# ChenWu98/cycle-diffusion

Measured on AMD Instinct MI355X. Metric: images/sec, SD-v1.4 512px CycleDiffusion 100+100 steps, 1/2/4/8 MI355X, higher is better.
Workload: dtype fp16; 1 GPU; C2: Stable-Diffusion-v1.4-shaped U-Net + KL-f8 VAE, 512x512, custom_steps=99 white_box_steps=100 eta=0.1 skip 0, 1 trial, encoder scale 1, decoder CFG 3; batch_per_gpu=4, global_batch=4, parallelism=dp1, steps_per_launch_set=5, launch_set_cap=16, launch_sets_in_flight_per_gpu=1, images_in_flight_per_gpu=20, distributed=single process, weights=synthetic(seed=0)

## Files before the change

### cycle-diffusion_amd/_ffi.py

```python
import ctypes as C
import os

import numpy as np

_HERE = os.path.dirname(os.path.abspath(__file__))
LIB_PATH = os.path.join(_HERE, "lib", "libcyclediff.so")

CD_NET_UNET_OPENAI, CD_NET_UNET_HO, CD_NET_VAE_KL, CD_NET_CLIP_TEXT, CD_NET_BERT_XTR = 1, 2, 3, 4, 5
CD_NET_OCLIP_TEXT, CD_NET_OCLIP_VISION, CD_NET_INCEPTION_FID, CD_NET_LPIPS = 6, 7, 8, 9
CD_SCHED_DDIM, CD_SCHED_DDPM = 0, 1
CD_PREC_16, CD_PREC_F32, CD_PREC_F32X3 = 0, 1, 2
CD_MASK_QSAMPLE, CD_MASK_ENCODER = 0, 1
MASK_SOURCES = {"q_sample": CD_MASK_QSAMPLE, "encoder": CD_MASK_ENCODER}
ACT_NONE, ACT_SILU, ACT_GELU, ACT_GEGLU, ACT_QGELU, ACT_RELU = 0, 1, 2, 3, 4, 5


class NetDesc(C.Structure):
    _fields_ = [
        ("kind", C.c_int), ("image_size", C.c_int), ("in_channels", C.c_int), ("out_channels", C.c_int),
        ("model_channels", C.c_int), ("num_res_blocks", C.c_int),
        ("n_mult", C.c_int), ("channel_mult", C.c_int * 8),
        ("n_attn", C.c_int), ("attn", C.c_int * 8),
        ("num_heads", C.c_int), ("num_head_channels", C.c_int),
        ("use_spatial_transformer", C.c_int), ("context_dim", C.c_int), ("transformer_depth", C.c_int),
# ... 78 lines not shown
    "cd_vae_encode": [_VP, _I, _VP, _VP, _U64, _I, _I, _I, _F, _VP],
    "cd_vae_decode": [_VP, _I, _VP, _I, _I, _F, _F, _F, _VP],
    "cd_vae_encode_hw": [_VP, _I, _VP, _VP, _U64, _I, _I, _I, _I, _F, _VP],
    "cd_vae_decode_hw": [_VP, _I, _VP, _I, _I, _I, _F, _F, _F, _VP],
    "cd_dpm_encode": [_VP, _I, _I, _VP, _VP, _VP, _I, _F, _I, _I, _VP, _VP, _U64, _I, _VP],
    "cd_ddim_decode": [_VP, _I, _I, _VP, _I, _I, _VP, _VP, _I, _F, _I, _I, _VP, _VP, _U64, _VP],
    "cd_ddim_decode_v": [_VP, _I, _I, _VP, _I, _I, _VP, _VP, _I, _VP, _I, _I, _VP, _VP, _U64, _VP],
    "cd_ddim_invert": [_VP, _I, _I, _VP, _VP, _VP, _I, _F, _I, _I, _VP, _VP, _VP],
    "cd_cycle_translate": [_VP, C.POINTER(TranslateArgs)],
    "cd_ddim_decode_masked": [_VP, _I, _I, _VP, _I, _I, _VP, _VP, _I, _F, _VP, _I, _I, _VP, _VP, _U64, _VP, _VP, _I, _I, _VP, _VP,
                              _U64, _VP],
    "cd_ilvr_decode": [_VP, _I, _I, _VP, _I, _I, _I, _I, _VP, _VP, _U64, _VP, _I, _I, _I, _VP, _VP, _U64, _VP],
    "cd_automask": [_VP, _I, _VP, _VP, _VP, _I, _I, _I, _I, _F, _F, _VP, _U64, _I, _F, _F, _I, _VP, _VP],
    "cd_word_maps": [_VP, _I, _VP, _VP, _I, _I, _VP, _I, _I, _I, _I, _F, _F, _VP, _U64, _I, _I, _I, _VP, C.POINTER(_I)],
    "cd_pix_refine": [_VP, _I, _I, _VP, _I, _I, _VP, _VP, _U64],
    "cd_op_pack_conv_weight": [_VP, _VP, _I, _I, _I, _I, _I, C.POINTER(_VP), C.POINTER(_I), C.POINTER(_I)],
    "cd_op_free": [_VP, _VP],
    "cd_op_conv2d": [_VP, _VP, _I, _VP, _I, _I, _I, _I, _VP, _I, _I, _I, _I, _I, _I, _I, _VP, _VP, _VP, _I, _I, _VP],
    "cd_op_conv2d_16": [_VP, _VP, _I, _VP, _I, _I, _I, _I, _VP, _I, _I, _I, _I, _I, _I, _I, _VP, _VP, _VP, _I, _I, _VP,
                        _VP],
    "cd_op_last_gemm_config": [_VP] + [C.POINTER(_I)] * 5,
    "cd_op_up_phase_reorder": [_VP, _VP, _I, _I, _I, _I, _VP],
    "cd_op_groupnorm": [_VP, _VP, _I, _I, _I, _I, _I, _F, _VP, _VP, _VP, _I, _VP],
    "cd_op_groupnorm_ex": [_VP, _VP, _I, _I, _VP, _I, _I, _I, _I, _I, _F, _VP, _VP, _VP, _I, _I, _VP, _VP, _I, _VP],
    "cd_op_pack_conv_weight_prec": [_VP, _VP, _I, _I, _I, _I, _I, C.POINTER(_VP)],
    "cd_op_conv2d_prec": [_VP, _VP, _I, _I, _VP, _I, _I, _I, _I, _I, _VP, _I, _I, _I, _I, _I, _I, _I, _VP, _VP, _I, _VP, _I, _I,
                          _I, _I, _I, _I, _F, _VP, _VP],
    "cd_op_attention_prec": [_VP, _VP, _VP, _VP, _I, _I, _I, _I, _I, _I, _I, _I, _F, _I, _VP, _I, _I, _VP],
    "cd_op_rows_prec": [_VP, _I, _VP, _I64, _I, _I, _VP, _I, _I, _VP, _VP, _I, _VP],
    "cd_op_resample_prec": [_VP, _I, _VP, _I, _I, _I, _I, _I, _VP],
    "cd_op_layernorm": [_VP, _VP, _I, _I, _VP, _VP, _F, _VP],
    "cd_op_st_entry": [_VP, _VP, _I, _I, _I, _VP, _VP, _F, _VP, _VP, _VP, _VP, _VP, _VP, _VP, _I, _VP, _VP, _VP,
                       C.POINTER(_I)],
    "cd_op_attention": [_VP, _VP, _VP, _VP, _I, _I, _I, _I, _I, _F, _I, _VP],
    "cd_op_cross_attention_ctrl": [_VP, _VP, _VP, _VP, _VP, _VP, _VP, _VP, _VP, _I, _I, _I, _I, _I, _I, _I, _I, _F, _VP],
    "cd_op_cross_attention_ctrl_ex": [_VP, _VP, _VP, _VP, _VP, _VP, _VP, _VP, _VP, _I, _I, _I, _I, _I, _I, _I, _I, _F, _I, _I,
                                      _VP],
    "cd_op_cross_attention_maps": [_VP, _VP, _VP, _VP, _I, _I, _I, _I, _I, _I, _I, _I, _F, _I, _VP],
    "cd_op_attention_ex": [_VP, _VP, _VP, _VP, _I, _I, _I, _I, _I, _I, _I, _I, _I, _I, _F, _I, _VP, _I, _I, _VP],
    "cd_op_lowpass": [_VP, _VP, _I, _I, _I, _I, _VP],
    "cd_op_softmax_rows": [_VP, _VP, _I64, _I, _VP],
    "cd_op_timestep_embedding": [_VP, _VP, _I, _I, _I, _VP],
    "cd_op_sched_step": [_VP, _I, _I, _VP, _VP, _VP, _VP, _I, _F, _VP, _VP, _I, _I, _I, _I, _VP],
    "cd_op_gauss": [_VP, _U64, C.c_uint32, _I64, _I64, _VP],
    "cd_op_automask_reduce": [_VP, _VP, _VP, _I, _I, _I, _I, _I, _F, _F, _I, _VP, _VP, _VP],
    "cd_op_local_blend_mask": [_VP, _VP, _VP, _I, _I, _I, _I, _I, _F, _VP],
    "cd_op_sched_step_masked": [_VP, _I, _VP, _VP, _VP, _I, _F, _VP, _VP, _VP, _I, _I, _F, _F, _VP, _I, _I, _I, _I, _VP, _I],
    "cd_op_sega_guidance": [_VP, _VP, _I, _I, _I, _I, _I, _F, _VP, _VP, _I, _F, _F, _VP, _VP, _VP, _VP, _VP],
    "cd_op_window_gather": [_VP, _VP, _VP, _I, _I, _I, _I, _I, _I, _I, _I, _VP],
    "cd_op_window_fuse": [_VP, _VP, _VP, _I, _I, _I, _I, _I, _I, _I, _I, _VP],
    "cd_op_layout": [_VP, _I, _VP, _VP, _I, _I, _I, _I, _I, _F, _F, _I],
    "cd_op_resample16": [_VP, _I, _VP, _VP, _I, _I, _I, _I],
    "cd_op_copy_rows16": [_VP, _VP, _I, _VP, _I, _I64, _I],
    "cd_op_vec_linear": [_VP, _VP, _I, _VP, _VP, _VP, _I, _I, _I, _I, _I, _I],
    "cd_op_tokens": [_VP, _I, _VP, _VP, _VP, _VP, _VP, _I, _I, _I, _I],
    "cd_op_posterior_sample": [_VP, _VP, _I, _VP, _U64, _VP, _I, _I, _I, _F, _I],
    "cd_op_vq_quantize": [_VP, _VP, _F, _VP, _I, _I, _I, _I, _VP, _I],
    "cd_op_gemm_batched": [_VP, _VP, _I, _I64, _VP, _I, _I64, _I, _I, _I, _I, _F, _VP, _VP, _I, _VP, _I, _I, _VP, _I, _I64, _I],
    "cd_op_attn_block_core": [_VP, _VP, _I, _VP, _I, _VP, _VP, _I, _I, _I, _VP, _I, _VP, C.POINTER(_I)],
    "cd_op_pool3x3": [_VP, _VP, _I, _I, _I, _I, _I, _I, _I, _I, _I, _I, _VP],
    "cd_op_global_avg": [_VP, _VP, _I, _I, _I, _I, _VP],
    "cd_op_basic_conv": [_VP, _VP, _I, _I, _I, _I, _I, _VP, _VP, _VP, _VP, _VP, _I, _I, _I, _I, _I, _I, _I, _I, _I, _VP, _VP,
                         _VP],
    "cd_op_lpips_layer": [_VP, _VP, _VP, _VP, _I, _I, _I, _I, _VP],
    "cd_op_pool2x2": [_VP, _VP, _I, _I, _I, _I, _I, _I, _I, _VP],
    "cd_op_bench_conv": [_VP, _I, _I, _I, _I, _I, _I, _I, _I, _I, _I, _I, _I, C.POINTER(C.c_float)],
# ... 53 lines not shown
```

### cycle-diffusion_amd/csrc/capi_internal.h

```cpp
#pragma once
#include <stdlib.h>
#include <string.h>
#include <unistd.h>

#include <map>
#include <utility>

#include "engine.h"

using namespace cd;

struct StepPacer {
  static constexpr int kAhead = 2, kRing = kAhead + 1;
  hipEvent_t ev[kRing] = {nullptr, nullptr, nullptr};
  long n = 0;
  bool enabled = true;
  void init() {
    const char* e = getenv("CYCLEDIFF_HOST_PACING");
    enabled = !(e && e[0] == '0');
    for (auto& x : ev) HIP_CHECK(hipEventCreateWithFlags(&x, hipEventBlockingSync | hipEventDisableTiming));
  }
  static void sleep_until_done(hipEvent_t e) {
    for (;;) {
      const hipError_t q = hipEventQuery(e);
// ... 15 lines not shown
    ++n;
  }
  void destroy() { for (auto& x : ev) if (x) { (void)hipEventDestroy(x); x = nullptr; } }
};

struct CoefStaging {
  static constexpr int kSlots = 4;
  static constexpr size_t kSlotBytes = 64 << 10;
  char* host = nullptr;
  hipEvent_t done[kSlots] = {nullptr, nullptr, nullptr, nullptr};
  int next = 0;
  void init() {
    HIP_CHECK(hipHostMalloc((void**)&host, kSlots * kSlotBytes, hipHostMallocDefault));
    for (auto& x : done) HIP_CHECK(hipEventCreateWithFlags(&x, hipEventBlockingSync | hipEventDisableTiming));
  }
  void destroy() {
    for (auto& x : done) if (x) { (void)hipEventDestroy(x); x = nullptr; }
    if (host) { (void)hipHostFree(host); host = nullptr; }
  }
};

struct cd_engine {
  hipStream_t st = nullptr;
  StepPacer pacer;
  CoefStaging coef_staging;
  Arena arena;
  bf16_t* zeros = nullptr;
  float* gn_partial = nullptr;
  size_t gn_partial_floats = 0;
  std::vector<std::unique_ptr<Net>> nets;
  std::vector<ParamStore*> op_stores;
  ParamStore op_params;
  std::map<std::pair<const void*, const void*>, std::pair<ConvW*, ConvW*>> op_st_entry;
  ParamStore op_params_f32;
  std::unique_ptr<KernelProfiler> prof;
  SplitKWorkspace splitk;
  int* overflow_host = nullptr;
  int* overflow_dev = nullptr;
  void check_overflow() {
    if (overflow_host && *(volatile int*)overflow_host) {
      *(volatile int*)overflow_host = 0;
      CD_CHECK(false, "CD_PREC_F32X3: a GroupNorm output or weight left the fp16 range of the split representation "
                      "(|x| >= 4094 or |w| >= 255); results since the last synchronisation are invalid - run this "
                      "network with CD_PREC_F32");
    }
  }
  Ctx ctx() {
    Ctx c; c.st = st; c.arena = &arena; c.zeros = zeros; c.gn_partial = gn_partial;
    c.gn_partial_floats = gn_partial_floats; c.overflow = overflow_dev;
    return c;
  }
};

struct ArenaScope {
  Arena& a;
  size_t m;
  explicit ArenaScope(Arena& arena) : a(arena), m(arena.mark()) {}
  ~ArenaScope() { a.release(m); }
  ArenaScope(const ArenaScope&) = delete;
  ArenaScope& operator=(const ArenaScope&) = delete;
};

void set_last_error(const char* what);

inline void enter_engine(cd_engine* h) {
  if (!h) return;
// ... 45 lines not shown
```

### cycle-diffusion_amd/csrc/capi_ops.hip

```cpp
#include "capi_internal.h"

namespace {

bf16_t* op_rows16(cd_engine* h, const float* src, int64_t rows, int C) {
  bf16_t* d = (bf16_t*)h->arena.alloc((size_t)rows * C * 2);
  launch_nchw_to_nhwc(h->st, src, d, (int)rows, C, 1, C, 1.f, 0.f, 0);
  return d;
}
Act op_image16(Ctx& c, const float* x, int B, int C, int H, int W, int Cpad) {
  Act a = alloc_act(c, B, H, W, Cpad);
  launch_nchw_to_nhwc(c.st, x, a.p, B, C, H * W, Cpad, 1.f, 0.f, 0);
  return a;
}

bf16_t* op_nan_rows16(cd_engine* h, int64_t rows, int ld) {
  const size_t bytes = (size_t)(rows + 64) * ld * 2;
  bf16_t* t = (bf16_t*)h->arena.alloc(bytes);
  HIP_CHECK(hipMemsetAsync(t, 0xFF, bytes, h->st));
  return t;
}
float* op_nan_buffer(cd_engine* h, size_t n) {
  float* t = (float*)h->arena.alloc(n * sizeof(float));
  launch_fill_f32(h->st, t, __builtin_nanf(""), (int64_t)n);
  return t;
// ... 279 lines not shown
               B > 0 && H > 0 && W > 0, "bad argument");
  ArenaScope arena_scope(h->arena);
  Ctx c = h->ctx();
  const int C = 320, T = H * W;
  ConvW win = *(const ConvW*)w_in;
  win.b = const_cast<float*>(b_in);
  StEntryW w;
  w.norm.g = const_cast<float*>(gn_gamma); w.norm.b = const_cast<float*>(gn_beta); w.norm.C = C; w.norm.eps = gn_eps;
  w.ln1.g = const_cast<float*>(ln_gamma); w.ln1.b = const_cast<float*>(ln_beta); w.ln1.C = C;
  w.proj_in = &win; w.qk1 = (const ConvW*)w_qk; w.v1 = (const ConvW*)w_v;
  CD_CHECK(win.N == C && win.Cpad == C && w.qk1->N == 2 * C && w.qk1->Cpad == C && w.v1->N == C && w.v1->Cpad == C,
           "transformer entry: 320-channel weights expected");
  w.vbias = v_bias;
  {
    const auto key = std::make_pair(w_qk, w_v);
    auto it = h->op_st_entry.find(key);
    if (it == h->op_st_entry.end()) {
      st_entry_alloc(h->op_params, w);
      it = h->op_st_entry.emplace(key, std::make_pair(w.qkv, w.qkv_ln)).first;
    }
    w.qkv = it->second.first; w.qkv_ln = it->second.second;
  }
  st_entry_refresh(h->st, w);
  Act a = op_image16(c, x, B, C, H, W, C);
  if (stages < 0) stages = st_entry_stages();
  const StEntryOut r = st_entry_fwd(c, w, a, stages);
  if (stages_run) *stages_run = r.stages;
  op_download_nchw(h, r.h.p, false, r.h.ld, h_out, B, C, T);
  op_download_nchw(h, r.qk.p, false, r.qk.ld, qk_out, B, 2 * C, T);
  op_download_nchw(h, r.vt, false, r.Tpad, vt_out, B * C, r.Tpad, 1);
  CD_API_END
}

int cd_op_attention(cd_handle h, const float* q, const float* k, const float* v, int B, int H, int Tq,
                    int Tk, int D, float scale, int use_transpose_kernel, float* o) {
  CD_API_BEGIN
  enter_engine(h);
  CD_CHECK(h && q && k && v && o, "bad argument");
  ArenaScope arena_scope(h->arena);
  const int C = H * D, Tpad = round_up(Tk, 64);
  const bf16_t* qb = op_rows16(h, q, (int64_t)B * Tq, C);
  const bf16_t* kb = op_rows16(h, k, (int64_t)B * Tk, C);
  const bf16_t* vb = op_rows16(h, v, (int64_t)B * Tk, C);
  bf16_t* ob = (bf16_t*)h->arena.alloc((size_t)B * Tq * C * 2);
  AttnParams p;
  p.q = qb; p.k = kb; p.o = ob; p.B = B; p.H = H; p.Tq = Tq; p.Tk = Tk; p.D = D;
  p.ldq = C; p.ldk = C; p.ldo = C; p.q_bs = (int64_t)Tq * C; p.k_bs = (int64_t)Tk * C; p.o_bs = (int64_t)Tq * C;
  p.scale = scale;
  if (use_transpose_kernel) {
    bf16_t* vt = (bf16_t*)h->arena.alloc((size_t)B * C * Tpad * 2);
    launch_transpose_v(h->st, vb, C, (int64_t)Tk * C, vt, B, H, Tk, D, D, Tpad);
    p.vt = vt; p.vt_dpad = D; p.vt_tpad = Tpad;
  } else {
    p.v = vb; p.ldv = C; p.v_bs = (int64_t)Tk * C;
  }
  launch_attention(h->st, p);
  op_download_nchw(h, ob, false, C, o, B * Tq, C, 1);
  CD_API_END
}

int cd_op_attention_ex(cd_handle h, const float* q, const float* k, const float* v, int B, int H, int Tq, int Tk, int D,
                       int layout, int pad, int v_transposed, int d_extra, int t_extra, float scale, int q_log2,
                       const float* obias, int causal, int opad, float* o) {
  CD_API_BEGIN
  enter_engine(h);
  CD_CHECK(h && q && k && v && o && B > 0 && H > 0 && Tq > 0 && Tk > 0 && D > 0 && D % 8 == 0, "bad argument");
// ... 841 lines not shown
```

### cycle-diffusion_amd/csrc/conv_gemm.hip

```cpp
#include <stdio.h>
#include <stdlib.h>
#include <string.h>

#include <algorithm>
#include <map>
#include <mutex>
#include <string>

#include "common.h"
#include "kernels.h"

namespace cd {

namespace gemm_detail {

typedef const __attribute__((address_space(1))) void* gptr_t;
typedef __attribute__((address_space(3))) void* lptr_t;

template <int BM, int BN, int BK, int WM, int WN, int NSTAGE>
struct TileCfg {
  static constexpr int NW = WM * WN;
  static constexpr int CPR = BK / 8;
  static constexpr int RPI = 64 / CPR;
  static constexpr int A_IPW = BM / RPI / NW;
// ... 1172 lines not shown
    }
    float v = 0.0f;
    if (np < N && c < Cin) v = w[(((int64_t)(n + src_row_offset) * Cin + c) * KH + r) * KW + s];
    out[i] = f2bf(v);
  }
}

__global__ void k_up_phase_weights(const bf16_t* __restrict__ w, bf16_t* __restrict__ out, int Npad, int Cpad) {
  const int64_t total = (int64_t)16 * Npad * Cpad;
  for (int64_t i = blockIdx.x * (int64_t)blockDim.x + threadIdx.x; i < total;
       i += (int64_t)gridDim.x * blockDim.x) {
    const int c = (int)(i % Cpad);
    int64_t t = i / Cpad;
    const int dx = (int)(t & 1), dy = (int)((t >> 1) & 1); t >>= 2;
    const int n = (int)(t % Npad);
    const int ph = (int)(t / Npad);
    const int a = ph >> 1, b = ph & 1;
    const int r0 = dy ? 1 + a : 0, r1 = dy ? 2 : a;
    const int s0 = dx ? 1 + b : 0, s1 = dx ? 2 : b;
    float v = 0.0f;
    for (int r = r0; r <= r1; ++r)
      for (int s = s0; s <= s1; ++s) v += bf2f(w[((int64_t)n * 9 + r * 3 + s) * Cpad + c]);
    out[i] = f2bf(v);
  }
}

void launch_up_phase_weights(hipStream_t st, const bf16_t* w, bf16_t* out, int Npad, int Cpad) {
  const int64_t total = (int64_t)16 * Npad * Cpad;
  int grid = (int)((total + 255) / 256);
  if (grid > 4096) grid = 4096;
  hipLaunchKernelGGL(k_up_phase_weights, dim3(grid), dim3(256), 0, st, w, out, Npad, Cpad);
}

void launch_repack_weight(hipStream_t st, const float* w, bf16_t* out, int N, int Cin, int KH,
                          int KW, int Npad, int Cpad, int geglu, int64_t src_row_offset) {
  const int64_t total = (int64_t)Npad * KH * KW * Cpad;
  int grid = (int)((total + 255) / 256);
  if (grid > 4096) grid = 4096;
  hipLaunchKernelGGL(k_repack_weight, dim3(grid), dim3(256), 0, st, w, out, N, Cin, KH, KW, Npad,
                     Cpad, geglu, src_row_offset);
}

}
```

### cycle-diffusion_amd/csrc/engine.h

```cpp
#pragma once
#include <map>
#include <memory>
#include <string>
#include <vector>

#include "common.h"
#include "kernels.h"
#include "../../include/cyclediff.h"

namespace cd {

class Arena {
 public:
  ~Arena();
  void init(size_t bytes);
  void* alloc(size_t bytes);
  size_t mark() const { return off_; }
  void release(size_t m) { off_ = m; }
  void reset() { off_ = 0; }
  size_t capacity() const { return cap_; }
  size_t high_water() const { return high_; }
 private:
  char* base_ = nullptr;
  size_t cap_ = 0, off_ = 0, high_ = 0;
// ... 152 lines not shown

struct AttnW {
  int C = 0, heads = 1;
  GNW norm;
  ConvW *qk = nullptr, *v = nullptr, *proj = nullptr;
  float* vbias = nullptr;
};
Act attn_block_fwd(Ctx& c, const AttnW& a, const Act& x);

enum {
  ST_ENTRY_QKV = 1,
  ST_ENTRY_LN1 = 2,
  ST_ENTRY_GN = 4,
};
int st_entry_stages();
bool st_entry_available(const Ctx& c, int64_t rows, int hw);
constexpr int64_t kStEntryNetMinRows = 61440;
struct StEntryW {
  GNW norm; LNW ln1;
  const ConvW *proj_in = nullptr, *qk1 = nullptr, *v1 = nullptr;
  ConvW *qkv = nullptr, *qkv_ln = nullptr;
  const float* vbias = nullptr;
};
void st_entry_alloc(ParamStore& ps, StEntryW& w);
void st_entry_refresh(hipStream_t st, StEntryW& w);
struct StEntryOut { Act h, qk; bf16_t* vt = nullptr; int Tpad = 0; int stages = 0; };
void vt_gemm_fwd(Ctx& c, const ConvW& wv, const bf16_t* x, int ldx, int B, int T, int Tpad, bf16_t* vt);
struct AtCoreOut { Act o; bf16_t* vt = nullptr; int Tpad = 0; int branch = 0; };
AtCoreOut at_core(Ctx& c, const ConvW& wv, const float* vbias, const Act& qk, const Act& n, int C, int heads, Act o = Act());
Act st_entry_proj_in(Ctx& c, const StEntryW& w, const Act& x, int stages);
StEntryOut st_entry_qkv(Ctx& c, const StEntryW& w, const Act& h, int stages);
StEntryOut st_entry_fwd(Ctx& c, const StEntryW& w, const Act& x, int stages);

Act avgpool2_fwd(Ctx& c, const Act& x);
Act upsample2_fwd(Ctx& c, const Act& x);
Act attention_f32_fwd(Ctx& c, const Act& qk, const Act& v, int H, int D, float scale, const float* obias);

Act attention_fwd(Ctx& c, const bf16_t* q, int ldq, const bf16_t* k, int ldk, const bf16_t* v, int ldv, int B,
                  int H, int Tq, int Tk, int D, float scale, int Himg, int Wimg, bool q_log2 = false, int rows = -1);
Act attention_vt_fwd(Ctx& c, const bf16_t* q, int ldq, const bf16_t* k, int ldk, const bf16_t* vt, int B,
                     int H, int Tq, int Tk, int Tpad, int D, float scale, int Himg, int Wimg, bool q_log2 = false,
                     const float* obias = nullptr, Act o = Act());

class Net {
 public:
  virtual ~Net() {}
  ParamStore params;
  cd_net_desc desc;
  bool f32 = false;
  bool x3 = false;
  void set_precision(const cd_net_desc& d) {
    f32 = d.precision == CD_PREC_F32 || d.precision == CD_PREC_F32X3;
    x3 = d.precision == CD_PREC_F32X3;
    params.f32 = f32; params.x3 = x3;
  }
  virtual int kind() const = 0;
};

struct TimeEmb {
  int mode = 0, dim = 0, hidden = 0;
  float *w0 = nullptr, *b0 = nullptr, *w1 = nullptr, *b1 = nullptr;
  float* proj_w = nullptr; float* proj_b = nullptr;
  int proj_total = 0;
};

struct AttnCtrl {
// ... 87 lines not shown
```

### cycle-diffusion_amd/csrc/engine.hip

```cpp
#include <limits.h>
#include <stdlib.h>

#include "engine.h"

#include <string.h>

namespace cd {

Arena::~Arena() { if (base_) (void)hipFree(base_); }
void Arena::init(size_t bytes) {
  if (base_) { (void)hipFree(base_); base_ = nullptr; }
  HIP_CHECK(hipMalloc((void**)&base_, bytes));
  cap_ = bytes; off_ = 0; high_ = 0;
}
void* Arena::alloc(size_t bytes) {
  size_t a = (off_ + 255) & ~(size_t)255;
  CD_CHECK(a + bytes <= cap_, "workspace arena exhausted: need %zu more bytes (capacity %zu); "
           "create the engine with a larger workspace", a + bytes - cap_, cap_);
  off_ = a + bytes;
  if (off_ > high_) high_ = off_;
  return base_ + a;
}

ParamStore::~ParamStore() {
// ... 414 lines not shown

int st_entry_stages() {
  static const int v = [] {
    const char* e = getenv("CYCLEDIFF_ST_ENTRY");
    int s = e && e[0] ? atoi(e) : (ST_ENTRY_QKV | ST_ENTRY_LN1 | ST_ENTRY_GN);
    if (!(s & ST_ENTRY_QKV)) s &= ~ST_ENTRY_LN1;
    return s;
  }();
  return v;
}

bool st_entry_available(const Ctx& c, int64_t rows, int hw) {
  return !c.f32 && rows >= 32768 && lin_stream_entry_supports(rows, hw, 320);
}

void st_entry_alloc(ParamStore& ps, StEntryW& w) {
  if (!w.qk1 || !w.v1 || !w.qk1->wfrag || !w.v1->wfrag || w.qk1->Cpad != 320 || w.qk1->N != 640 || w.v1->N != 320) return;
  w.qkv = ps.new_conv(960, 320, 1, 1, true);
  w.qkv_ln = ps.new_conv(960, 320, 1, 1, true);
}

void st_entry_refresh(hipStream_t st, StEntryW& w) {
  if (!w.qkv) return;
  const size_t row = (size_t)320 * sizeof(bf16_t);
  HIP_CHECK(hipMemcpyAsync(w.qkv->w, w.qk1->w, 640 * row, hipMemcpyDeviceToDevice, st));
  HIP_CHECK(hipMemcpyAsync(w.qkv->w + (size_t)640 * 320, w.v1->w, 320 * row, hipMemcpyDeviceToDevice, st));
  HIP_CHECK(hipMemsetAsync(w.qkv->b, 0, 960 * sizeof(float), st));
  if (w.vbias) HIP_CHECK(hipMemcpyAsync(w.qkv->b + 640, w.vbias, 320 * sizeof(float), hipMemcpyDeviceToDevice, st));
  launch_pack_wfrag(st, w.qkv->w, 320, w.qkv->wfrag, 960);
  if (w.ln1.g && w.qkv_ln) {
    launch_fold_ln(st, w.qkv->w, 320, w.ln1.g, w.ln1.b, w.qkv->b, w.qkv_ln->w, w.qkv_ln->b, 960, 320);
    launch_pack_wfrag(st, w.qkv_ln->w, 320, w.qkv_ln->wfrag, 960);
  }
}

void vt_gemm_fwd(Ctx& c, const ConvW& wv, const bf16_t* x, int ldx, int B, int T, int Tpad, bf16_t* vt) {
  ConvGemmParams p;
  p.src0 = wv.w; p.C0 = wv.Cpad; p.ld0 = wv.Cpad;
  p.B = 1; p.Hs = wv.N; p.Ws = 1; p.Hin = wv.N; p.Win = 1; p.Hout = wv.N; p.Wout = 1;
  p.M = wv.N;
  p.wgt = x; p.Ktot = wv.Cpad; p.ldw = ldx; p.N = T;
  p.nbatch = B; p.a_bs = 0; p.w_bs = (int64_t)T * ldx; p.o_bs = (int64_t)wv.N * Tpad;
  p.out = vt; p.out_ld = Tpad; p.zeros = c.zeros;
  launch_conv_gemm(c.st, p);
}

int st_entry_effective(const Ctx& c, const StEntryW& w, const Act& x, int stages) {
  const bool fused_ok = w.qkv && w.norm.C == 320 && x.C == 320 && x.ld == 320 && st_entry_available(c, x.rows(), x.H * x.W);
  if (!fused_ok) stages = 0;
  if (!(stages & ST_ENTRY_QKV) || !w.qkv_ln || !conv_ln_fold_available(c, *w.qkv_ln, x.rows())) stages &= ~ST_ENTRY_LN1;
  return stages;
}

Act st_entry_proj_in(Ctx& c, const StEntryW& w, const Act& x, int stages) {
  const int B = x.B, T = x.H * x.W, C = w.norm.C;
  ConvOpts p0; p0.pad = 0;
  stages = st_entry_effective(c, w, x, stages);
  Act h;
  if (stages & ST_ENTRY_GN) {
    const float* coef = groupnorm_coef_fwd(c, w.norm, x);
    h = alloc_act(c, B, x.H, x.W, C);
    launch_lin_stream_gn(c.st, x.p, x.ld, (int)x.rows(), T, coef, w.proj_in->wfrag, w.proj_in->b, h.p, h.ld);
  } else {
    Act n = groupnorm_fwd(c, w.norm, x, nullptr, false);
    h = conv_fwd(c, *w.proj_in, n, nullptr, p0);
  }
// ... 292 lines not shown
```

### cycle-diffusion_amd/csrc/kernels.h

```cpp
#pragma once
#include <map>
#include <string>
#include <vector>

#include "common.h"

namespace cd {

struct StepCoef {
  float sa, s1a, sap, dirc, sigma, r, t_mask;
  int t;
};
enum { SCHED_DDIM = 0, SCHED_DDPM = 1 };

struct EpsHat {
  const float* p = nullptr;
  int64_t sb = 0, sc = 0, sp = 0;
  int cfg = 0;
  float g = 1.f;
  const float* gvec = nullptr;
};

struct StepGeom {
  int B = 0, C = 0, HW = 0;
// ... 202 lines not shown
  int out_f32 = 0;
  float* stats = nullptr;
  const bf16_t* zeros = nullptr;
  int ln_fold = 0;
  float ln_eps = 1e-5f;
  int tile = 0;
  float prof_flop_scale = 1.f;
  int splitk = 0;
  float* sk_scratch = nullptr;
  int* sk_flags = nullptr;
  int korder = 1;
  int tile_group = 0;
  int up_phase = 0;
  int w_ps = 0;
};
struct SplitKWorkspace {
  float* scratch = nullptr;
  size_t scratch_bytes = 0;
  int* flags = nullptr;
  int nflags = 0;
};
extern thread_local SplitKWorkspace g_conv_splitk;
void launch_conv_gemm(hipStream_t st, const ConvGemmParams& p);
const char* conv_gemm_last_config();
struct GemmLaunchInfo {
  int tile_id = 0;
  int bk = 0;
  int splitk = 1;
  int chm = 0;
  int tile_group = 0;
};
GemmLaunchInfo conv_gemm_last_launch();
void launch_up_phase_weights(hipStream_t st, const bf16_t* w, bf16_t* out, int Npad, int Cpad);
int conv_gemm_num_configs();
const char* conv_gemm_config_name(int id);

struct LinStreamParams {
  const bf16_t* a = nullptr; int lda = 0;
  const bf16_t* wfrag = nullptr;
  const float* bias = nullptr;
  const bf16_t* resid = nullptr; int ldr = 0;
  bf16_t* out = nullptr; int ldo = 0;
  float* stats = nullptr;
  int M = 0, N = 0;
  float ln_eps = 1e-5f;
  int nsplit = 0, hw = 0;
  bf16_t* vt = nullptr; int vt_ld = 0;
  int64_t vt_bytes = 0;
  const float* gn_coef = nullptr;
};
constexpr int kLinStreamTile = 30;
bool lin_stream_supports(const ConvGemmParams& p);
void launch_lin_stream(hipStream_t st, const ConvGemmParams& p);
bool lin_stream_entry_supports(int64_t M, int hw, int lda);
void launch_lin_stream_qkv(hipStream_t st, const bf16_t* a, int lda, int M, int hw, const bf16_t* wfrag, const float* bias,
                           bf16_t* qk, bf16_t* vt, int vt_ld, bool ln_fold, float ln_eps);
void launch_lin_stream_gn(hipStream_t st, const bf16_t* a, int lda, int M, int hw, const float* gn_coef, const bf16_t* wfrag,
                          const float* bias, bf16_t* out, int ldo);
void launch_fold_ln(hipStream_t st, const bf16_t* w, int ldw, const float* gamma, const float* beta, const float* bias,
                    bf16_t* w_out, float* bias_out, int N, int Kc);
void launch_pack_wfrag(hipStream_t st, const bf16_t* w, int ldw, bf16_t* out, int N);

struct KernelProfiler {
  bool enabled = false;
  std::vector<hipEvent_t> events;
  std::vector<double> flops;
// ... 168 lines not shown
```

### cycle-diffusion_amd/csrc/unet_openai.hip

```cpp
#include <algorithm>

#include "engine.h"

namespace cd {

namespace {

struct STW {
  int C = 0, heads = 0, dh = 0, ctx = 0;
  GNW norm;
  ConvW *proj_in = nullptr, *proj_out = nullptr;
  LNW ln1, ln2, ln3;
  ConvW *qkv1 = nullptr, *qk1 = nullptr, *v1 = nullptr, *o1 = nullptr;
  ConvW *q2 = nullptr, *k2 = nullptr, *v2 = nullptr, *o2 = nullptr;
  ConvW *ff1 = nullptr, *ff2 = nullptr;
  ConvW *q2_ln = nullptr, *ff1_ln = nullptr;
  StEntryW entry;
  int side = 0;
  bf16_t* k2c = nullptr;
  bf16_t* v2c = nullptr;
};

struct Layer {
  enum Kind { CONV_IN, RES, ST, AB, DOWN_CONV, UP_CONV } kind;
  int idx = 0;
  ConvW* conv = nullptr;
};
struct Block { std::vector<Layer> layers; };

class UNetOpenAI : public UNet {
 public:
  explicit UNetOpenAI(const cd_net_desc& d);
  int kind() const override { return CD_NET_UNET_OPENAI; }
  void forward(Ctx& c, const UNetIO& io) override;
  void set_context(Ctx& c, const bf16_t* ctx, int B, int L) override;
  void build_attn_control(Ctx& c, const float* mapper, const float* alpha, const float* weight, int B_ctrl,
                          AttnCtrl& ctrl) override;
  int count_text_blocks(int min_side, int max_side) const override;
  size_t workspace_hint(int B) const override;

 private:
  int mc_, hidden_;
  TimeEmb te_;
  std::vector<ResW> res_;
  std::vector<STW> st_;
  std::vector<AttnW> ab_;
  std::vector<Block> in_blocks_, out_blocks_;
  Block mid_;
  GNW out_norm_;
// ... 35 lines not shown
  s.norm = make_gn(params, pfx + ".norm", C, 1e-6f);
  s.proj_in = make_conv(params, pfx + ".proj_in", C, C, 1, true);
  s.proj_out = make_conv(params, pfx + ".proj_out", C, C, 1, true);
  const std::string tb = pfx + ".transformer_blocks.0";
  s.ln1 = make_ln(params, tb + ".norm1", C);
  s.ln2 = make_ln(params, tb + ".norm2", C);
  s.ln3 = make_ln(params, tb + ".norm3", C);
  const float qscale = 1.44269504088896340736f / sqrtf((float)dh);
  if (dh == 40) {
    s.qk1 = params.new_conv(2 * C, C, 1, 1, false);
    params.conv_rows(tb + ".attn1.to_q.weight", {C, C}, s.qk1, 0, C, 0, C, 0, qscale);
    params.conv_rows(tb + ".attn1.to_k.weight", {C, C}, s.qk1, C, C, 0, C, 0);
    s.v1 = make_conv(params, tb + ".attn1.to_v", C, C, 1, false, false, 2);
    s.entry.norm = s.norm; s.entry.ln1 = s.ln1;
    s.entry.proj_in = s.proj_in; s.entry.qk1 = s.qk1; s.entry.v1 = s.v1;
    st_entry_alloc(params, s.entry);
  } else {
    s.qkv1 = params.new_conv(3 * C, C, 1, 1, false);
    params.conv_rows(tb + ".attn1.to_q.weight", {C, C}, s.qkv1, 0, C, 0, C, 0, qscale);
    params.conv_rows(tb + ".attn1.to_k.weight", {C, C}, s.qkv1, C, C, 0, C, 0);
    params.conv_rows(tb + ".attn1.to_v.weight", {C, C}, s.qkv1, 2 * C, C, 0, C, 0);
  }
  s.o1 = make_conv(params, tb + ".attn1.to_out.0", C, C, 1, true, false, 2);
  s.q2 = make_conv(params, tb + ".attn2.to_q", C, C, 1, false, false, 2, qscale);
  s.k2 = make_conv(params, tb + ".attn2.to_k", C, s.ctx, 1, false, false, 2);
  s.v2 = make_conv(params, tb + ".attn2.to_v", C, s.ctx, 1, false, false, 2);
  s.o2 = make_conv(params, tb + ".attn2.to_out.0", C, C, 1, true, false, 2);
  s.ff1 = make_conv(params, tb + ".ff.net.0.proj", 8 * C, C, 1, true, true, 2);
  s.ff2 = make_conv(params, tb + ".ff.net.2", C, 4 * C, 1, true, false, 2);
  if (s.q2->wfrag) {
    s.q2_ln = params.new_conv(C, C, 1, 1, true);
    s.ff1_ln = params.new_conv(8 * C, C, 1, 1, true, true);
  }
  st_.push_back(s);
  return (int)st_.size() - 1;
}

int UNetOpenAI::add_ab(const std::string& pfx, int C, int heads) {
  AttnW a; a.C = C; a.heads = heads;
  a.norm = make_gn(params, pfx + ".norm", C, 1e-5f);
  const int ch = C / heads;
  a.qk = params.new_conv(2 * C, C, 1, 1, true);
  a.v = params.new_conv(C, C, 1, 1, false);
  a.vbias = params.new_vec(C);
  const std::string wn = pfx + ".qkv.weight", bn = pfx + ".qkv.bias";
  params.conv_rows(wn, {3 * C, C, 1}, a.qk, 0, C, 0, ch, 3 * ch);
  params.conv_rows(wn, {3 * C, C, 1}, a.qk, C, C, ch, ch, 3 * ch);
  params.conv_rows(wn, {3 * C, C, 1}, a.v, 0, C, 2 * ch, ch, 3 * ch);
  params.bias_rows(bn, 3 * C, a.qk->b, 0, C, 0, ch, 3 * ch);
  params.bias_rows(bn, 3 * C, a.qk->b, C, C, ch, ch, 3 * ch);
  params.bias_rows(bn, 3 * C, a.vbias, 0, C, 2 * ch, ch, 3 * ch);
  a.proj = make_conv(params, pfx + ".proj_out", C, C, 1, true, false, 3);
  ab_.push_back(a);
  return (int)ab_.size() - 1;
}

UNetOpenAI::UNetOpenAI(const cd_net_desc& d) {
  desc = d;
  set_precision(d);

  mc_ = d.model_channels; hidden_ = 4 * mc_;
  image_size = d.image_size; out_channels = d.out_channels;
  in_cpad = round_up(d.in_channels, 32);
  CD_CHECK(mc_ % 32 == 0, "model_channels must be a multiple of 32");
  const bool use_st = d.use_spatial_transformer != 0;
  auto has_attn = [&](int ds) { for (int i = 0; i < d.n_attn; ++i) if (d.attn[i] == ds) return true; return false; };
// ... 332 lines not shown
        launch_word_map_accumulate(c.st, ma);
      }
      ++maps_->layers;
      ++maps_->seen;
    } else if (maps_ && maps_->takes(x.H)) {
      CD_CHECK(x.H == x.W && x.H == s.side && B == maps_->n_chunk * maps_->B, "word maps: block of side %d, %d rows", x.H, B);
      WordMapParams mp;
      mp.q = q.p; mp.k = s.k2c; mp.sel = maps_->sel;
      mp.maps = (float*)c.arena->alloc((size_t)B * maps_->N * T * 4);
      mp.B = B; mp.B_sel = maps_->B_sel; mp.H = s.heads; mp.Tq = T; mp.L = ctx_L_; mp.D = s.dh; mp.N = maps_->N;
      mp.ldq = q.ld; mp.ldk = C; mp.q_bs = (int64_t)T * q.ld; mp.k_bs = (int64_t)ctx_L_ * C;
      mp.scale = scale; mp.q_log2 = 1;
      launch_cross_attention_maps(c.st, mp);
      WordMapAccum ma;
      ma.layer = mp.maps; ma.acc = maps_->acc; ma.rows = B; ma.N = maps_->N; ma.s = x.H; ma.h = image_size; ma.w = image_size;
      ma.first = maps_->layers == 0 ? 1 : 0;
      launch_word_map_accumulate(c.st, ma);
      ++maps_->layers;
    }
    ConvOpts o; o.pad = 0; o.resid = &h; o.out = h.p; o.out_ld = h.ld;
    conv_fwd(c, *s.o2, a, nullptr, o);
    c.arena->release(m2);
  }
  {
    const size_t m2 = c.arena->mark();
    Act g;
    if (s.ff1_ln && conv_ln_fold_available(c, *s.ff1_ln, h.rows())) {
      ConvOpts pl; pl.pad = 0; pl.ln_fold = true;
      g = conv_fwd(c, *s.ff1_ln, h, nullptr, pl);
    } else {
      Act n3 = layernorm_fwd(c, s.ln3, h);
      g = conv_fwd(c, *s.ff1, n3, nullptr, p0);
    }
    ConvOpts o; o.pad = 0; o.resid = &h; o.out = h.p; o.out_ld = h.ld;
    conv_fwd(c, *s.ff2, g, nullptr, o);
    c.arena->release(m2);
  }
  ConvOpts po; po.pad = 0; po.resid = &x; po.out = out.p; po.out_ld = out.ld; po.out_stats = out.stats_buf;
  conv_fwd(c, *s.proj_out, h, nullptr, po);
  c.arena->release(mk);
}

Act UNetOpenAI::run_block(Ctx& c, const Block& b, Act h, const Act* skip, const float* proj, int proj_ld,
                          bool t_shared) {
  bool first = true;
  for (const Layer& l : b.layers) {
    const Act* x2 = first ? skip : nullptr;
    switch (l.kind) {
      case Layer::CONV_IN: { ConvOpts o; o.want_stats = true; h = conv_fwd(c, *l.conv, h, nullptr, o); break; }
      case Layer::RES: h = res_fwd(c, res_[l.idx], h, x2, proj, proj_ld, t_shared); break;
      case Layer::ST: h = st_fwd(c, st_[l.idx], h); break;
      case Layer::AB: h = attn_block_fwd(c, ab_[l.idx], h); break;
      case Layer::DOWN_CONV: { ConvOpts o; o.stride = 2; o.want_stats = true; h = conv_fwd(c, *l.conv, h, nullptr, o); break; }
      case Layer::UP_CONV: { ConvOpts o; o.up = true; o.want_stats = true; h = conv_fwd(c, *l.conv, h, nullptr, o); break; }
    }
    first = false;
  }
  return h;
}

void UNetOpenAI::refresh_ln_folds(Ctx& c) {
  if (folded_version_ == params.version) return;
  for (const Block& b : out_blocks_)
    for (const Layer& l : b.layers)
      if (l.kind == Layer::UP_CONV) params.refresh_up_phase(c.st, l.conv);
  for (STW& s : st_) {
    st_entry_refresh(c.st, s.entry);
    if (!s.q2_ln) continue;
    struct { const ConvW* src; ConvW* dst; const LNW* ln; } jobs[2] = {{s.q2, s.q2_ln, &s.ln2}, {s.ff1, s.ff1_ln, &s.ln3}};
    for (auto& j : jobs) {
      launch_fold_ln(c.st, j.src->w, j.src->Ktot(), j.ln->g, j.ln->b, j.src->b, j.dst->w, j.dst->b, j.src->Npad,
                     j.src->Cpad);
      launch_pack_wfrag(c.st, j.dst->w, j.dst->Ktot(), j.dst->wfrag, j.dst->Npad);
    }
  }
  folded_version_ = params.version;
}

void UNetOpenAI::forward(Ctx& c, const UNetIO& io) {
  const size_t mk0 = c.arena->mark();
  PrecisionScope prec(c, f32, x3);
  refresh_ln_folds(c);
  CD_CHECK(!io.ctrl || (!f32 && io.ctrl->va.size() == st_.size()), "U-Net: cross-attention control on a network it was not built for");
  CD_CHECK(!io.maps || !f32, "U-Net: per-word attention maps are not built for fp32 / fp32x3 networks (their transformer blocks "
           "run the fp32 attention of st_f32.hip): use the 16-bit precision");
  const bool maps_all = io.maps && !io.maps->ranged();
  CD_CHECK(!(maps_all && io.ctrl), "U-Net: a forward collects per-word attention maps or runs cross-attention control, not both");
  CD_CHECK(!maps_all || (io.dup_tail == 0 && !io.cfg_dup), "U-Net: per-word attention maps on a batch with repeated rows");
  ctrl_ = io.ctrl;
  maps_ = io.maps;
  if (maps_) maps_->layers = 0;
  const int B = io.B, R = image_size;
  const float* proj = time_emb_fwd(c, te_, io);
  const int proj_ld = te_.proj_total;
  const Act x = net_input_act(io.xin, B, R, R, in_cpad, f32, x3);
  std::vector<Act> hs;
  Act h = x;
  size_t first_full = 0;
  static const bool cfg_share = [] { const char* e = getenv("CYCLEDIFF_CFG_SHARE"); return !(e && e[0] == '0'); }();
  CD_CHECK(!(io.cfg_dup && io.dup_tail) && io.dup_tail >= 0 && 2 * io.dup_tail <= B, "U-Net: repeated-row description");
// ... 47 lines not shown
```

### include/cyclediff.h

```cpp
#ifndef CYCLEDIFF_H
#define CYCLEDIFF_H
#include <stddef.h>
#include <stdint.h>

#ifdef __cplusplus
extern "C" {
#endif

typedef struct cd_engine* cd_handle;

enum { CD_NET_UNET_OPENAI = 1, CD_NET_UNET_HO = 2, CD_NET_VAE_KL = 3, CD_NET_CLIP_TEXT = 4, CD_NET_BERT_XTR = 5,
       CD_NET_OCLIP_TEXT = 6, CD_NET_OCLIP_VISION = 7, CD_NET_INCEPTION_FID = 8, CD_NET_LPIPS = 9 };
enum { CD_SCHED_DDIM = 0, CD_SCHED_DDPM = 1 };
enum { CD_PREC_16 = 0, CD_PREC_F32 = 1, CD_PREC_F32X3 = 2 };
enum { CD_MASK_QSAMPLE = 0, CD_MASK_ENCODER = 1 };

typedef struct cd_net_desc {
  int kind;
  int image_size;
  int in_channels, out_channels;
  int model_channels;
  int num_res_blocks;
  int n_mult;  int channel_mult[8];
  int n_attn;  int attn[8];
// ... 180 lines not shown
int cd_op_free(cd_handle h, void* dev);
int cd_op_conv2d(cd_handle h, const float* x0, int C0, const float* x1, int C1, int B, int H, int W,
                 const void* packed_w, int N, int KH, int KW, int stride, int pad, int asym_pad, int up,
                 const float* bias, const float* rowvec, const float* resid, int act, int tile, float* y);
int cd_op_conv2d_16(cd_handle h, const float* x0, int C0, const float* x1, int C1, int B, int H, int W,
                    const void* packed_w, int N, int KH, int KW, int stride, int pad, int asym_pad, int up,
                    const float* bias, const float* rowvec, const float* resid, int act, int tile, float* y,
                    float* stats);
int cd_op_last_gemm_config(cd_handle h, int* tile_id, int* bk, int* splitk, int* chm, int* tile_group);
int cd_op_up_phase_reorder(cd_handle h, const float* x, int B, int C, int H, int W, float* y);
int cd_op_groupnorm(cd_handle h, const float* x, int B, int C, int H, int W, int G, float eps,
                    const float* gamma, const float* beta, const float* film, int silu, float* y);
int cd_op_groupnorm_ex(cd_handle h, const float* x0, int C0, int pad0, const float* x1, int C1, int pad1, int B, int H,
                       int W, float eps, const float* gamma, const float* beta, const float* film, int film_ld, int silu,
                       const float* stats0, const float* stats1, int precision, void* y);
int cd_op_pack_conv_weight_prec(cd_handle h, const float* w_host, int N, int Cin, int KH, int KW, int geglu,
                                void** packed_dev);
int cd_op_conv2d_prec(cd_handle h, const float* x0, int C0, int pad0, const float* x1, int C1, int pad1, int B, int H, int W,
                      const void* packed_w, int N, int KH, int KW, int stride, int pad, int asym_pad, int up,
                      const float* bias, const float* rowvec, int rowvec_shared, const float* resid, int resid_pad, int act,
                      int raw_geglu, int tile, int precision, int via_split_rows, float alpha, float* y, float* stats);
int cd_op_attention_prec(cd_handle h, const float* q, const float* k, const float* v, int B, int H, int Tq, int Tk, int D,
                         int padq, int padk, int padv, float scale, int q_log2, const float* obias, int mode, int precision,
                         void* o);
int cd_op_rows_prec(cd_handle h, int op, const float* x0, int64_t rows, int C0, int pad0, const float* x1, int C1, int pad1,
                    const float* gamma, const float* beta, int precision, void* y);
int cd_op_resample_prec(cd_handle h, int op, const float* x, int B, int C, int H, int W, int precision, void* y);
int cd_op_layernorm(cd_handle h, const float* x, int rows, int C, const float* gamma, const float* beta,
                    float eps, float* y);
int cd_op_st_entry(cd_handle h, const float* x, int B, int H, int W, const float* gn_gamma, const float* gn_beta,
                   float gn_eps, const void* w_in, const float* b_in, const float* ln_gamma, const float* ln_beta,
                   const void* w_qk, const void* w_v, const float* v_bias, int stages, float* h_out, float* qk_out,
                   float* vt_out, int* stages_run);
int cd_op_attention(cd_handle h, const float* q, const float* k, const float* v, int B, int H, int Tq,
                    int Tk, int D, float scale, int use_transpose_kernel, float* o);
int cd_op_cross_attention_ctrl(cd_handle h, const float* q_own, const float* q_src, const float* k_own, const float* k_src,
                               const float* v_own, const float* mapper, const float* alpha, const float* weight, int B,
                               int B_src, int B_ctrl, int H, int Tq, int L, int L_buf, int D, float scale, float* o);
int cd_op_cross_attention_ctrl_ex(cd_handle h, const float* q_own, const float* q_src, const float* k_own, const float* k_src,
                                  const float* v_own, const float* mapper, const float* alpha, const float* weight, int B,
                                  int B_src, int B_ctrl, int H, int Tq, int L, int L_buf, int D, float scale, int q_log2,
                                  int opad, float* o);
int cd_op_cross_attention_maps(cd_handle h, const float* q, const float* k, const float* sel, int B, int B_sel, int H,
                               int Tq, int L, int L_buf, int D, int N, float scale, int q_log2, float* maps );
int cd_op_attention_ex(cd_handle h, const float* q, const float* k, const float* v, int B, int H, int Tq, int Tk, int D,
                       int layout, int pad, int v_transposed, int d_extra, int t_extra, float scale, int q_log2,
                       const float* obias, int causal, int opad, float* o);
int cd_op_lowpass(cd_handle h, const float* x, int B, int C, int R, int down_n, float* y);
int cd_op_softmax_rows(cd_handle h, const float* s, int64_t rows, int cols, float* p);
int cd_op_timestep_embedding(cd_handle h, const float* t, int B, int dim, int mode, float* out);
int cd_op_sched_step(cd_handle h, int mode, int sched_kind, const cd_step_coef* coef_host, const float* x0,
                     float* xt, const float* eps_hat, int cfg, float guidance, const float* noise,
                     const float* eps_in, int is_last, int B, int C, int HW, float* z_slot);
int cd_op_gauss(cd_handle h, uint64_t seed, uint32_t stream, int64_t first, int64_t n, float* out);
int cd_op_automask_reduce(cd_handle h, const float* eps_src, const float* eps_tgt, int n, int B, int C, int H, int W,
                          float ratio, float thr, int dilate, float* map_out, float* mean_out, float* keep_out);
int cd_op_local_blend_mask(cd_handle h, const float* acc_src, const float* acc_tgt, int B, int Bd, int side, int f, int pool,
                           float thr, float* keep_out);
int cd_op_window_gather(cd_handle h, const float* x, const int32_t* win_host, int n_win, int Bp, int C, int Hc, int Wc, int S,
                        int cpad, int dup, float* y_out);
int cd_op_window_fuse(cd_handle h, const float* e, const int32_t* win_host, int n_win, int Bp, int C, int Hc, int Wc, int S,
                      int ld, int parts, float* out);
int cd_op_sched_step_masked(cd_handle h, int mode, const cd_step_coef* coef_host, float* x, const float* eps_hat, int cfg,
                            float guidance, const float* eps_in, const float* mask, const float* src, int B_mask,
                            int mask_source, float qa, float qb, const float* mask_noise, int blend, int B, int C, int HW,
                            void* xin16_out, int cfg_dup);
// ... 40 lines not shown
```

Before: 3.593 images/s.

## Fold transformer ff2 and proj_out GEMMs into one concatenated-K GEMM

Precomputes a combined weight [W_po*W_ff2 | W_po] and bias so that the feed-forward output projection and the transformer proj_out run as a single GEMM over the concatenated [g, h] input. This removes one GEMM launch and the write and reread of the intermediate residual activation. The folded product is rounded to bf16, which changes numerics slightly. The fold is enabled by default for channel widths up to 640 and can be controlled with an environment mask.

```diff
diff --git a/cycle-diffusion_amd/_ffi.py b/cycle-diffusion_amd/_ffi.py
--- a/cycle-diffusion_amd/_ffi.py
+++ b/cycle-diffusion_amd/_ffi.py
@@ -134,6 +134,7 @@
     "cd_op_layernorm": [_VP, _VP, _I, _I, _VP, _VP, _F, _VP],
     "cd_op_st_entry": [_VP, _VP, _I, _I, _I, _VP, _VP, _F, _VP, _VP, _VP, _VP, _VP, _VP, _VP, _I, _VP, _VP, _VP,
                        C.POINTER(_I)],
+    "cd_op_st_tail": [_VP, _VP, _VP, _VP, _I, _I, _I, _I, _VP, _VP, _VP, _VP, _I, _I, _VP, _VP, C.POINTER(_I)],
     "cd_op_attention": [_VP, _VP, _VP, _VP, _I, _I, _I, _I, _I, _F, _I, _VP],
     "cd_op_cross_attention_ctrl": [_VP, _VP, _VP, _VP, _VP, _VP, _VP, _VP, _VP, _I, _I, _I, _I, _I, _I, _I, _I, _F, _VP],
     "cd_op_cross_attention_ctrl_ex": [_VP, _VP, _VP, _VP, _VP, _VP, _VP, _VP, _VP, _I, _I, _I, _I, _I, _I, _I, _I, _F, _I, _I,
diff --git a/cycle-diffusion_amd/csrc/capi_internal.h b/cycle-diffusion_amd/csrc/capi_internal.h
--- a/cycle-diffusion_amd/csrc/capi_internal.h
+++ b/cycle-diffusion_amd/csrc/capi_internal.h
@@ -71,6 +71,7 @@
   std::vector<ParamStore*> op_stores;
   ParamStore op_params;
   std::map<std::pair<const void*, const void*>, std::pair<ConvW*, ConvW*>> op_st_entry;
+  std::map<std::pair<const void*, const void*>, ConvW*> op_st_tail;
   ParamStore op_params_f32;
   std::unique_ptr<KernelProfiler> prof;
   SplitKWorkspace splitk;
diff --git a/cycle-diffusion_amd/csrc/capi_ops.hip b/cycle-diffusion_amd/csrc/capi_ops.hip
--- a/cycle-diffusion_amd/csrc/capi_ops.hip
+++ b/cycle-diffusion_amd/csrc/capi_ops.hip
@@ -335,6 +335,46 @@
   CD_API_END
 }
 
+int cd_op_st_tail(cd_handle h, const float* g, const float* h2, const float* x, int B, int H, int W, int C,
+                  const void* w_ff2, const float* b_ff2, const void* w_po, const float* b_po, int fold, int tile,
+                  float* out, float* stats, int* fold_ran) {
+  CD_API_BEGIN
+  enter_engine(h);
+  CD_CHECK(h && g && h2 && x && w_ff2 && w_po && out && B > 0 && H > 0 && W > 0 && C > 0 && C % 32 == 0, "bad argument");
+  ArenaScope arena_scope(h->arena);
+  Ctx c = h->ctx();
+  ConvW ff2 = *(const ConvW*)w_ff2, po_w = *(const ConvW*)w_po;
+  CD_CHECK(ff2.N == C && ff2.Cpad == 4 * C && po_w.N == C && po_w.Cpad == C, "transformer tail: C x 4C and C x C weights expected");
+  ff2.b = const_cast<float*>(b_ff2);
+  po_w.b = const_cast<float*>(b_po);
+  ConvW* tail = nullptr;
+  if (fold) {
+    const auto key = std::make_pair(w_ff2, w_po);
+    auto it = h->op_st_tail.find(key);
+    if (it == h->op_st_tail.end()) it = h->op_st_tail.emplace(key, st_tail_alloc(h->op_params, ff2, po_w)).first;
+    tail = it->second;
+    CD_CHECK(tail, "transformer tail: no derived weight for these layers");
+    st_tail_refresh(h->st, ff2, po_w, *tail);
+  }
+  const int64_t rows = (int64_t)B * H * W;
+  Act ga = op_rows_view(op_rows16(h, g, rows, 4 * C), B, H * W, 4 * C, 4 * C, false);
+  Act ha = op_rows_view(op_rows16(h, h2, rows, C), B, H * W, C, C, false);
+  Act xa = op_rows_view(op_rows16(h, x, rows, C), B, H * W, C, C, false);
+  ga.H = ha.H = xa.H = H; ga.W = ha.W = xa.W = W;
+  Act o = alloc_act(c, B, H, W, C);
+  ConvOpts po; po.pad = 0; po.resid = &xa; po.out = o.p; po.out_ld = o.ld;
+  const bool with_stats = (H * W) % 32 == 0;
+  if (with_stats) po.out_stats = (float*)h->arena.alloc((size_t)(rows / 32) * 2 * C * sizeof(float));
+  CD_CHECK(!stats || with_stats, "transformer tail: statistics need H*W %% 32 == 0");
+  if (tail && st_tail_fold_on(C)) po.tile = tile;
+  const bool ran = st_tail_fwd(c, ff2, po_w, tail, ga, ha, po);
+  if (fold_ran) *fold_ran = ran ? 1 : 0;
+  op_download_nchw(h, o.p, false, o.ld, out, (int)rows, C, 1);
+  if (stats)
+    HIP_CHECK(hipMemcpyAsync(stats, po.out_stats, (size_t)(rows / 32) * 2 * C * sizeof(float), hipMemcpyDeviceToDevice, h->st));
+  CD_API_END
+}
+
 int cd_op_attention(cd_handle h, const float* q, const float* k, const float* v, int B, int H, int Tq,
                     int Tk, int D, float scale, int use_transpose_kernel, float* o) {
   CD_API_BEGIN
diff --git a/cycle-diffusion_amd/csrc/conv_gemm.hip b/cycle-diffusion_amd/csrc/conv_gemm.hip
--- a/cycle-diffusion_amd/csrc/conv_gemm.hip
+++ b/cycle-diffusion_amd/csrc/conv_gemm.hip
@@ -1228,6 +1228,41 @@
   hipLaunchKernelGGL(k_up_phase_weights, dim3(grid), dim3(256), 0, st, w, out, Npad, Cpad);
 }
 
+__global__ void k_st_tail_weights(const bf16_t* __restrict__ w_po, const bf16_t* __restrict__ w_ff2,
+                                  const float* __restrict__ b_po, const float* __restrict__ b_ff2,
+                                  bf16_t* __restrict__ out, float* __restrict__ bias_out, int C) {
+  const int K4 = 4 * C, K5 = 5 * C;
+  const int k = blockIdx.x * blockDim.x + threadIdx.x;
+  const int n0 = blockIdx.y * 4;
+  if (k < K4) {
+    float acc[4] = {0.f, 0.f, 0.f, 0.f};
+    for (int j = 0; j < C; ++j) {
+      const float f = bf2f(w_ff2[(int64_t)j * K4 + k]);
+#pragma unroll
+      for (int r = 0; r < 4; ++r) acc[r] = fmaf(bf2f(w_po[(int64_t)(n0 + r) * C + j]), f, acc[r]);
+    }
+#pragma unroll
+    for (int r = 0; r < 4; ++r) out[(int64_t)(n0 + r) * K5 + k] = f2bf(acc[r]);
+  } else if (k < K5) {
+#pragma unroll
+    for (int r = 0; r < 4; ++r) out[(int64_t)(n0 + r) * K5 + k] = w_po[(int64_t)(n0 + r) * C + (k - K4)];
+  }
+  if (k < 4 && bias_out) {
+    const int n = n0 + k;
+    float acc = b_po ? b_po[n] : 0.f;
+    if (b_ff2)
+      for (int j = 0; j < C; ++j) acc = fmaf(bf2f(w_po[(int64_t)n * C + j]), b_ff2[j], acc);
+    bias_out[n] = acc;
+  }
+}
+
+void launch_st_tail_weights(hipStream_t st, const bf16_t* w_po, const bf16_t* w_ff2, const float* b_po, const float* b_ff2,
+                            bf16_t* out, float* bias_out, int C) {
+  CD_CHECK(C > 0 && C % 32 == 0, "transformer tail: %d channels", C);
+  hipLaunchKernelGGL(k_st_tail_weights, dim3((5 * C + 255) / 256, C / 4), dim3(256), 0, st, w_po, w_ff2, b_po, b_ff2, out,
+                     bias_out, C);
+}
+
 void launch_repack_weight(hipStream_t st, const float* w, bf16_t* out, int N, int Cin, int KH,
                           int KW, int Npad, int Cpad, int geglu, int64_t src_row_offset) {
   const int64_t total = (int64_t)Npad * KH * KW * Cpad;
diff --git a/cycle-diffusion_amd/csrc/engine.h b/cycle-diffusion_amd/csrc/engine.h
--- a/cycle-diffusion_amd/csrc/engine.h
+++ b/cycle-diffusion_amd/csrc/engine.h
@@ -208,6 +208,13 @@
 StEntryOut st_entry_qkv(Ctx& c, const StEntryW& w, const Act& h, int stages);
 StEntryOut st_entry_fwd(Ctx& c, const StEntryW& w, const Act& x, int stages);
 
+constexpr int kStTailFoldDefault = 3;
+ConvW* st_tail_alloc(ParamStore& ps, const ConvW& ff2, const ConvW& proj_out);
+void st_tail_refresh(hipStream_t st, const ConvW& ff2, const ConvW& proj_out, ConvW& tail);
+bool st_tail_fold_on(int C);
+bool st_tail_fwd(Ctx& c, const ConvW& ff2, const ConvW& proj_out, const ConvW* tail, const Act& g, const Act& h,
+                 const ConvOpts& po);
+
 Act avgpool2_fwd(Ctx& c, const Act& x);
 Act upsample2_fwd(Ctx& c, const Act& x);
 Act attention_f32_fwd(Ctx& c, const Act& qk, const Act& v, int H, int D, float scale, const float* obias);
diff --git a/cycle-diffusion_amd/csrc/engine.hip b/cycle-diffusion_amd/csrc/engine.hip
--- a/cycle-diffusion_amd/csrc/engine.hip
+++ b/cycle-diffusion_amd/csrc/engine.hip
@@ -470,6 +470,36 @@
     launch_fold_ln(st, w.qkv->w, 320, w.ln1.g, w.ln1.b, w.qkv->b, w.qkv_ln->w, w.qkv_ln->b, 960, 320);
     launch_pack_wfrag(st, w.qkv_ln->w, 320, w.qkv_ln->wfrag, 960);
   }
+}
+
+ConvW* st_tail_alloc(ParamStore& ps, const ConvW& ff2, const ConvW& proj_out) {
+  const int C = proj_out.N;
+  if (ps.f32 || C % 32 != 0 || proj_out.Cpad != C || proj_out.KH != 1 || proj_out.KW != 1 || ff2.N != C || ff2.Cpad != 4 * C ||
+      ff2.KH != 1 || ff2.KW != 1 || ff2.geglu || proj_out.geglu)
+    return nullptr;
+  return ps.new_conv(C, 5 * C, 1, 1, true);
+}
+
+void st_tail_refresh(hipStream_t st, const ConvW& ff2, const ConvW& proj_out, ConvW& tail) {
+  launch_st_tail_weights(st, proj_out.w, ff2.w, proj_out.b, ff2.b, tail.w, tail.b, proj_out.N);
+}
+
+bool st_tail_fold_on(int C) {
+  const char* e = getenv("CYCLEDIFF_ST_TAIL_FOLD");
+  const int mask = e && e[0] ? atoi(e) : kStTailFoldDefault;
+  return (mask >> (C <= 320 ? 0 : C <= 640 ? 1 : 2)) & 1;
+}
+
+bool st_tail_fwd(Ctx& c, const ConvW& ff2, const ConvW& proj_out, const ConvW* tail, const Act& g, const Act& h,
+                 const ConvOpts& po) {
+  if (tail && !c.f32 && st_tail_fold_on(proj_out.N)) {
+    conv_fwd(c, *tail, g, &h, po);
+    return true;
+  }
+  ConvOpts o; o.pad = 0; o.resid = &h; o.out = h.p; o.out_ld = h.ld;
+  conv_fwd(c, ff2, g, nullptr, o);
+  conv_fwd(c, proj_out, h, nullptr, po);
+  return false;
 }
 
 void vt_gemm_fwd(Ctx& c, const ConvW& wv, const bf16_t* x, int ldx, int B, int T, int Tpad, bf16_t* vt) {
diff --git a/cycle-diffusion_amd/csrc/kernels.h b/cycle-diffusion_amd/csrc/kernels.h
--- a/cycle-diffusion_amd/csrc/kernels.h
+++ b/cycle-diffusion_amd/csrc/kernels.h
@@ -258,6 +258,8 @@
 };
 GemmLaunchInfo conv_gemm_last_launch();
 void launch_up_phase_weights(hipStream_t st, const bf16_t* w, bf16_t* out, int Npad, int Cpad);
+void launch_st_tail_weights(hipStream_t st, const bf16_t* w_po, const bf16_t* w_ff2, const float* b_po, const float* b_ff2,
+                            bf16_t* out, float* bias_out, int C);
 int conv_gemm_num_configs();
 const char* conv_gemm_config_name(int id);
 
diff --git a/cycle-diffusion_amd/csrc/unet_openai.hip b/cycle-diffusion_amd/csrc/unet_openai.hip
--- a/cycle-diffusion_amd/csrc/unet_openai.hip
+++ b/cycle-diffusion_amd/csrc/unet_openai.hip
@@ -15,6 +15,7 @@
   ConvW *q2 = nullptr, *k2 = nullptr, *v2 = nullptr, *o2 = nullptr;
   ConvW *ff1 = nullptr, *ff2 = nullptr;
   ConvW *q2_ln = nullptr, *ff1_ln = nullptr;
+  ConvW* tail = nullptr;
   StEntryW entry;
   int side = 0;
   bf16_t* k2c = nullptr;
@@ -116,6 +117,7 @@
     s.q2_ln = params.new_conv(C, C, 1, 1, true);
     s.ff1_ln = params.new_conv(8 * C, C, 1, 1, true, true);
   }
+  s.tail = st_tail_alloc(params, *s.ff2, *s.proj_out);
   st_.push_back(s);
   return (int)st_.size() - 1;
 }
@@ -514,12 +516,10 @@
       Act n3 = layernorm_fwd(c, s.ln3, h);
       g = conv_fwd(c, *s.ff1, n3, nullptr, p0);
     }
-    ConvOpts o; o.pad = 0; o.resid = &h; o.out = h.p; o.out_ld = h.ld;
-    conv_fwd(c, *s.ff2, g, nullptr, o);
+    ConvOpts po; po.pad = 0; po.resid = &x; po.out = out.p; po.out_ld = out.ld; po.out_stats = out.stats_buf;
+    st_tail_fwd(c, *s.ff2, *s.proj_out, s.tail, g, h, po);
     c.arena->release(m2);
   }
-  ConvOpts po; po.pad = 0; po.resid = &x; po.out = out.p; po.out_ld = out.ld; po.out_stats = out.stats_buf;
-  conv_fwd(c, *s.proj_out, h, nullptr, po);
   c.arena->release(mk);
 }
 
@@ -548,6 +548,7 @@
       if (l.kind == Layer::UP_CONV) params.refresh_up_phase(c.st, l.conv);
   for (STW& s : st_) {
     st_entry_refresh(c.st, s.entry);
+    if (s.tail) st_tail_refresh(c.st, *s.ff2, *s.proj_out, *s.tail);
     if (!s.q2_ln) continue;
     struct { const ConvW* src; ConvW* dst; const LNW* ln; } jobs[2] = {{s.q2, s.q2_ln, &s.ln2}, {s.ff1, s.ff1_ln, &s.ln3}};
     for (auto& j : jobs) {
diff --git a/include/cyclediff.h b/include/cyclediff.h
--- a/include/cyclediff.h
+++ b/include/cyclediff.h
@@ -236,6 +236,9 @@
                    float gn_eps, const void* w_in, const float* b_in, const float* ln_gamma, const float* ln_beta,
                    const void* w_qk, const void* w_v, const float* v_bias, int stages, float* h_out, float* qk_out,
                    float* vt_out, int* stages_run);
+int cd_op_st_tail(cd_handle h, const float* g, const float* h2, const float* x, int B, int H, int W, int C,
+                  const void* w_ff2, const float* b_ff2, const void* w_po, const float* b_po, int fold, int tile,
+                  float* out, float* stats, int* fold_ran);
 int cd_op_attention(cd_handle h, const float* q, const float* k, const float* v, int B, int H, int Tq,
                     int Tk, int D, float scale, int use_transpose_kernel, float* o);
 int cd_op_cross_attention_ctrl(cd_handle h, const float* q_own, const float* q_src, const float* k_own, const float* k_src,
```

Result: no change. 3.619 images/s, median of 6 (+0.7%).
